# jojolebarjos/board-game-simulator-python

Hardware: AMD Instinct MI355X
Metric: env-steps/sec, Connect4(6,7,4) random rollout, batch=2^20 per GPU (higher is better)
Workload: dtype u64

## Files before the change

### board-game-simulator-python_amd/csrc/bgs_host.hip

```cpp
#include <immintrin.h>
#include <limits.h>
#include <linux/futex.h>
#include <pthread.h>
#include <sched.h>
#include <sys/syscall.h>
#include <time.h>
#include <unistd.h>

#include <atomic>
#include <chrono>
#include <condition_variable>
#include <cstdlib>
#include <cstdio>
#include <algorithm>
#include <cstring>
#include <mutex>
#include <new>
#include <thread>
#include <vector>

#include "bgs_capi_util.h"
#include "bgs_common.h"
#include "bgs_internal.h"

struct bgs_event {
    int device;
    hipEvent_t ev;
};

namespace {

using bgs::fail;

struct ExpandTable {
    uint64_t pairs[256];
    ExpandTable() {
        for (int byte = 0; byte < 256; ++byte) {
            uint64_t four = 0;
            for (int j = 0; j < 4; ++j) four |= (uint64_t)bgs::reward_pair((uint32_t)(byte >> (2 * j)) & 3u) << (16 * j);
            pairs[byte] = four;
        }
    }
};
const ExpandTable g_expand;

template <bool STREAM>
__attribute__((target("avx2"))) int64_t expand_avx2(const uint8_t* src, int64_t code_bytes, int8_t* dst) {
    const __m256i spread = _mm256_setr_epi8(0, 0, 0, 0, 1, 1, 1, 1, 2, 2, 2, 2, 3, 3, 3, 3,
                                            4, 4, 4, 4, 5, 5, 5, 5, 6, 6, 6, 6, 7, 7, 7, 7);
    const __m256i field = _mm256_set1_epi32((int)0xC0300C03u);
    const __m256i one = _mm256_set1_epi32(0x40100401);
    const __m256i two = _mm256_set1_epi32((int)0x80200802u);
    int64_t i = 0;
    for (; i + 8 <= code_bytes; i += 8) {
        long long eight;
        memcpy(&eight, src + i, 8);
        const __m256i rep = _mm256_shuffle_epi8(_mm256_set1_epi64x(eight), spread);
        const __m256i f = _mm256_and_si256(rep, field);
        const __m256i is1 = _mm256_cmpeq_epi8(f, one), is2 = _mm256_cmpeq_epi8(f, two);
        const __m256i r0 = _mm256_sub_epi8(is2, is1), r1 = _mm256_sub_epi8(is1, is2);
        const __m256i lo = _mm256_unpacklo_epi8(r0, r1), hi = _mm256_unpackhi_epi8(r0, r1);
        const __m256i first = _mm256_permute2x128_si256(lo, hi, 0x20), second = _mm256_permute2x128_si256(lo, hi, 0x31);
        if (STREAM) {
            _mm256_stream_si256(reinterpret_cast<__m256i*>(dst + 8 * i), first);
            _mm256_stream_si256(reinterpret_cast<__m256i*>(dst + 8 * i + 32), second);
        } else {
            _mm256_storeu_si256(reinterpret_cast<__m256i*>(dst + 8 * i), first);
            _mm256_storeu_si256(reinterpret_cast<__m256i*>(dst + 8 * i + 32), second);
        }
    }
    if (STREAM) _mm_sfence();
    return i;
}

const bool g_have_avx2 = __builtin_cpu_supports("avx2");
const bool g_stream_stores = bgs::experiment("no_stream_stores") == nullptr;

void expand_range(const uint8_t* packed, int64_t first, int64_t count, int8_t* reward) {
    const int64_t whole = count / 4;
    const uint8_t* src = packed + first / 4;
    int8_t* out = reward + 2 * first;
    int64_t i0 = 0;
    if (g_have_avx2) {
        const bool stream = (reinterpret_cast<uintptr_t>(out) & 31u) == 0 && whole >= (1 << 14) && g_stream_stores;
        i0 = stream ? expand_avx2<true>(src, whole, out) : expand_avx2<false>(src, whole, out);
    }
    for (int64_t i = i0; i < whole; ++i) memcpy(out + 8 * i, &g_expand.pairs[src[i]], 8);
    for (int64_t g = first + whole * 4; g < first + count; ++g) {
        const uint16_t pair = bgs::reward_pair((uint32_t)(packed[g / 4] >> (2 * (g & 3))) & 3u);
        memcpy(reward + 2 * g, &pair, 2);
    }
}

struct CellFormat {
    int cells = 0;
    int nwc = 0;
    int sets = 0;
    int offset = 0;
    int weight[4] = {0, 0, 0, 0};
};

struct SpreadTable {
    uint64_t v[256];
    SpreadTable() {
        for (int byte = 0; byte < 256; ++byte) {
            uint64_t w = 0;
            for (int b = 0; b < 8; ++b) w |= (uint64_t)((byte >> b) & 1) << (8 * b);
            v[byte] = w;
        }
    }
};
const SpreadTable g_spread;

__attribute__((target("avx512f,avx512bw"))) void expand_cells_avx512(const uint64_t* wire, int64_t n, const CellFormat& f,
                                                                      int64_t first, int64_t count, int8_t* out) {
    const __m512i base = _mm512_set1_epi8((char)f.offset);
    __m512i weight[4];
    for (int p = 0; p < f.sets; ++p) weight[p] = _mm512_set1_epi8((char)f.weight[p]);
    alignas(64) int8_t block[64 * 256 + 64];
    const bool lines = f.cells <= 256 && g_stream_stores && (reinterpret_cast<uintptr_t>(out) & 63u) == 0;
#define BGS_ONE_GAME(i_)                                                                                              \
    do {                                                                                                                \
        int8_t* dst_ = out + (i_)*f.cells;                                                                              \
        for (int j = 0; j < f.nwc; ++j) {                                                                               \
// ... 87 lines not shown
    if (!f) return false;
    int node = -1;
    const int got = fscanf(f, "%d", &node);
    fclose(f);
    if (got != 1 || node < 0) return false;
    snprintf(path, sizeof path, "/sys/devices/system/node/node%d/cpulist", node);
    f = fopen(path, "r");
    if (!f) return false;
    char list[4096] = {0};
    const bool have = fgets(list, sizeof list, f) != nullptr;
    fclose(f);
    if (!have) return false;
    cpu_set_t allowed;
    if (sched_getaffinity(0, sizeof allowed, &allowed) != 0) return false;
    int any = 0;
    char* save = nullptr;
    for (char* tok = strtok_r(list, ",\n", &save); tok; tok = strtok_r(nullptr, ",\n", &save)) {
        int lo = 0, hi = 0;
        const int k = sscanf(tok, "%d-%d", &lo, &hi);
        if (k < 1) continue;
        if (k == 1) hi = lo;
        for (int c = lo; c <= hi && c < CPU_SETSIZE; ++c)
            if (CPU_ISSET(c, &allowed)) {
                CPU_SET(c, out);
                ++any;
            }
    }
    return any > 0;
}

}

namespace {
inline bool sink_trace_on() {
    static const bool on = bgs::experiment("sink_trace") != nullptr;
    return on;
}
inline double mono_us() {
    return std::chrono::duration<double, std::micro>(std::chrono::steady_clock::now().time_since_epoch()).count();
}
}

static bool codes_hold_a_zero(const uint8_t* codes, int64_t first, int64_t count) {
    const uint8_t* p = codes + first / 4;
    const int64_t whole = count / 4;
    int64_t i = 0;
    uint64_t seen = 0;
    for (; i + 8 <= whole; i += 8) {
        uint64_t x;
        memcpy(&x, p + i, 8);
        seen |= ~(x | (x >> 1)) & 0x5555555555555555ull;
    }
    for (; i < whole; ++i) seen |= (uint64_t)(~(p[i] | (p[i] >> 1)) & 0x55u);
    for (int64_t k = 0; k < count - whole * 4; ++k) seen |= ((p[whole] >> (2 * k)) & 3u) == 0u ? 1u : 0u;
    return seen != 0;
}

struct bgs_reward_sink {
    int device = 0;
    int64_t max_games = 0;
    int slots = 0;
    int ring = 0;
    int threads = 0;
    std::vector<uint8_t*> pinned;
    std::vector<uint8_t*> mapped;
    std::vector<hipEvent_t> landed;
    bool grids = false;
    CellFormat cells;
    size_t slot_bytes = 0;
    struct Job {
        int64_t n_games = 0;
        int8_t* host_reward = nullptr;
        int event_slot = 0;
        bool all_end = false;
    };
    std::vector<Job> jobs;
    std::mutex mu;
    std::condition_variable cv_submit;
    std::condition_variable cv_landed;
    std::condition_variable cv_done;
    int64_t claimed = 0;
    int64_t submitted = 0;
    volatile int64_t* progress = nullptr;
    int64_t landed_upto = 0;
    int64_t completed = 0;
    std::vector<int> parts_done;
    std::vector<char> slot_ok;
    bool stop = false;
    std::vector<int64_t> failed_tickets;
    bool poll = false;
    std::vector<std::thread> workers;
    std::atomic<int64_t> a_submitted{0}, a_landed{0}, a_completed{0};
    std::atomic<bool> a_stop{false};
    std::atomic<int> urgent{0};
    int spin_us = 0;
    int wait_spin_us = 200;

    bool spin_for(const std::atomic<int64_t>& counter, int64_t ticket) const {
        if (counter.load(std::memory_order_acquire) > ticket) return true;
        if (spin_us <= 0) return false;
        const auto until = std::chrono::steady_clock::now() + std::chrono::microseconds(spin_us);
        for (;;) {
            for (int i = 0; i < 64; ++i) {
                if (counter.load(std::memory_order_acquire) > ticket || a_stop.load(std::memory_order_relaxed)) return true;
                _mm_pause();
            }
            if (std::chrono::steady_clock::now() >= until) return false;
        }
    }

    void work(int t) {
        (void)hipSetDevice(device);
        for (int64_t ticket = 0;; ++ticket) {
            const int slot = (int)(ticket % ring);
            Job job;
            bool ok = true;
            if (t == 0) {
                spin_for(a_submitted, ticket);
                {
                    std::unique_lock<std::mutex> lock(mu);
                    cv_submit.wait(lock, [&] { return stop || submitted > ticket; });
                    if (submitted <= ticket) return;
                    job = jobs[slot];
                }
                if (job.n_games == 0) {
                    ok = false;
                } else if (poll || urgent.load(std::memory_order_relaxed) > 0) {
                    hipError_t e;
                    while ((e = hipEventQuery(landed[job.event_slot])) == hipErrorNotReady) _mm_pause();
                    ok = e == hipSuccess;
                } else {
                    ok = hipEventSynchronize(landed[job.event_slot]) == hipSuccess;
                }
                if (sink_trace_on()) fprintf(stderr, "sink-trace ticket %lld landed %.1f\n", (long long)ticket, mono_us());
                {
                    std::lock_guard<std::mutex> lock(mu);
                    if (!ok && job.n_games != 0) failed_tickets.push_back(ticket);
                    slot_ok[slot] = ok;
                    landed_upto = ticket + 1;
                    a_landed.store(ticket + 1, std::memory_order_release);
                }
                cv_landed.notify_all();
            } else {
                if (urgent.load(std::memory_order_relaxed) > 0) {
                    const auto until = std::chrono::steady_clock::now() + std::chrono::microseconds(2000);
                    while (a_landed.load(std::memory_order_acquire) <= ticket && !a_stop.load(std::memory_order_relaxed) &&
                           urgent.load(std::memory_order_relaxed) > 0 && std::chrono::steady_clock::now() < until)
                        for (int i = 0; i < 16; ++i) _mm_pause();
                } else {
                    spin_for(a_landed, ticket);
                }
                std::unique_lock<std::mutex> lock(mu);
                cv_landed.wait(lock, [&] { return stop || landed_upto > ticket; });
                if (landed_upto <= ticket) return;
                job = jobs[slot];
                ok = slot_ok[slot];
            }
            const int expanders = threads > 1 ? threads - 1 : 1;
            const int share = threads > 1 ? t - 1 : 0;
            if (threads > 1 && t == 0) continue;
            const double trace_t0 = sink_trace_on() ? mono_us() : 0.0;
            if (ok && grids) {
                const int64_t blocks = (job.n_games + 63) / 64;
                const int64_t g0 = blocks * share / expanders * 64;
                const int64_t g1 = share + 1 == expanders ? job.n_games : blocks * (share + 1) / expanders * 64;
                static const bool skip = bgs::experiment("grid_no_expand") != nullptr;
                if (g1 > g0 && !skip) expand_cells(pinned[slot], job.n_games, cells, g0, g1 - g0, job.host_reward);
            } else if (ok) {
                const int64_t bytes = (job.n_games + 3) / 4;
                const int64_t b0 = bytes * share / expanders, b1 = bytes * (share + 1) / expanders;
                const int64_t first = b0 * 4;
                int64_t count = b1 * 4 - first;
                if (first + count > job.n_games) count = job.n_games - first;
                if (count > 0) expand_range(pinned[slot], first, count, job.host_reward);
                if (count > 0 && job.all_end && codes_hold_a_zero(pinned[slot], first, count)) {
                    std::lock_guard<std::mutex> lock(mu);
                    if (std::find(failed_tickets.begin(), failed_tickets.end(), ticket) == failed_tickets.end()) failed_tickets.push_back(ticket);
                }
            }
            if (sink_trace_on()) fprintf(stderr, "sink-trace ticket %lld worker %d expand %.1f .. %.1f\n", (long long)ticket, t, trace_t0, mono_us());
            {
                std::lock_guard<std::mutex> lock(mu);
                if (++parts_done[slot] == expanders) {
                    parts_done[slot] = 0;
                    ++completed;
                    a_completed.store(completed, std::memory_order_release);
                    cv_done.notify_all();
                    if (progress) progress_store_max(progress, completed);
                }
            }
        }
    }
};

namespace {

int64_t claim(bgs_reward_sink* s, bool ahead = false) {
    const int bound = ahead ? s->ring : s->slots;
    s->spin_for(s->a_completed, s->a_submitted.load(std::memory_order_relaxed) - bound);
    std::unique_lock<std::mutex> lock(s->mu);
    s->cv_done.wait(lock, [&] { return s->claimed - s->completed < bound; });
    return s->claimed++;
}

void publish(bgs_reward_sink* s, int64_t ticket, int64_t n_games, int8_t* host_reward, bool ok = true, int64_t event_ticket = -1,
             bool all_end = false) {
    {
        std::unique_lock<std::mutex> lock(s->mu);
        s->cv_done.wait(lock, [&] { return s->submitted == ticket; });
        s->jobs[ticket % s->ring].n_games = ok ? n_games : 0;
        s->jobs[ticket % s->ring].all_end = all_end;
        s->jobs[ticket % s->ring].host_reward = host_reward;
        s->jobs[ticket % s->ring].event_slot = (int)((event_ticket >= 0 ? event_ticket : ticket) % s->ring);
        if (!ok) s->failed_tickets.push_back(ticket);
        s->submitted = ticket + 1;
        s->a_submitted.store(ticket + 1, std::memory_order_release);
    }
    s->cv_submit.notify_one();
    s->cv_done.notify_all();
}

}

namespace bgs {
int64_t sink_claim(bgs_reward_sink* s) { return claim(s); }
uint8_t* sink_slot_device(bgs_reward_sink* s, int64_t ticket) { return s->mapped[ticket % s->ring]; }
uint8_t* sink_slot_host(bgs_reward_sink* s, int64_t ticket) { return s->pinned[ticket % s->ring]; }
hipEvent_t sink_slot_event(bgs_reward_sink* s, int64_t ticket) { return s->landed[ticket % s->ring]; }
void sink_publish(bgs_reward_sink* s, int64_t ticket, int64_t n_games, int8_t* host_reward, bool ok, int64_t event_ticket, bool all_end) {
    publish(s, ticket, n_games, host_reward, ok, event_ticket, all_end);
}
bool sink_takes_group(const bgs_reward_sink* s, int count) { return s != nullptr && !s->grids && count <= s->ring; }
int sink_ring(const bgs_reward_sink* s) { return s->ring; }
int sink_rollout_group(bgs_reward_sink* s, bgs_batch* const* bs, const uint64_t* seeds, const bool* writes, int count,
                       hipStream_t stream, int8_t* const* host_rewards, int64_t* tickets) {
    NEED(count >= 1 && count <= kConnectGroupMax && count <= s->ring && !s->grids, "bad step group");
    for (int i = 0; i < count; ++i)
        NEED(bs[i]->device == s->device && bs[i]->n <= s->max_games, "the batch does not fit the sink");
    uint32_t* codes[kConnectGroupMax];
    for (int i = 0; i < count; ++i) {
        tickets[i] = claim(s, true);
        codes[i] = reinterpret_cast<uint32_t*>(s->mapped[tickets[i] % s->ring]);
    }
    connect_rollout_steps(bs, seeds, codes, writes, count, stream);
    hipError_t err = hipGetLastError();
    if (err == hipSuccess) err = hipEventRecord(s->landed[tickets[count - 1] % s->ring], stream);
    for (int i = 0; i < count; ++i) publish(s, tickets[i], bs[i]->n, host_rewards[i], err == hipSuccess, tickets[count - 1]);
    if (err != hipSuccess) return fail(BGS_ERR_RUNTIME, "grouped rollout could not be enqueued: %s", hipGetErrorString(err));
    return BGS_OK;
}
int sink_wait(bgs_reward_sink* s, int64_t ticket, bool urgent) {
    NEED(s != nullptr, "sink is NULL");
    NEED(ticket >= 0 && ticket < s->a_submitted.load(std::memory_order_acquire), "unknown ticket %lld", (long long)ticket);
    if (s->a_completed.load(std::memory_order_acquire) <= ticket) {
        if (urgent) {
            s->urgent.fetch_add(1, std::memory_order_relaxed);
            const auto until = std::chrono::steady_clock::now() + std::chrono::microseconds(s->wait_spin_us);
            while (s->a_completed.load(std::memory_order_acquire) <= ticket && std::chrono::steady_clock::now() < until)
                for (int i = 0; i < 32; ++i) _mm_pause();
        } else {
            s->spin_for(s->a_completed, ticket);
        }
        {
            std::unique_lock<std::mutex> lock(s->mu);
            s->cv_done.wait(lock, [&] { return s->completed > ticket; });
        }
        if (urgent) s->urgent.fetch_sub(1, std::memory_order_relaxed);
    }
    int64_t bad = -1;
    {
        std::lock_guard<std::mutex> lock(s->mu);
        auto& f = s->failed_tickets;
        for (size_t i = 0; i < f.size();) {
            if (f[i] <= ticket) {
                if (bad < 0 || f[i] < bad) bad = f[i];
                f.erase(f.begin() + (long)i);
            } else {
                ++i;
            }
        }
    }
    if (bad >= 0)
        return fail(BGS_ERR_RUNTIME, "reward hand-over %lld failed (its enqueue, its arrival event, or -- a gathered step whose games all "
                    "had to end -- a rank delivered games that are still running: its step failed there); later deliveries are unaffected",
                    (long long)bad);
    return BGS_OK;
}
}

extern "C" {

int bgs_host_alloc(size_t bytes, void** host_ptr) {
    NEED(host_ptr != nullptr && bytes > 0, "bad argument");
    *host_ptr = nullptr;
    HIP_TRY(hipHostMalloc(host_ptr, bytes, hipHostMallocDefault));
    return BGS_OK;
}

int bgs_host_free(void* host_ptr) {
    if (host_ptr) HIP_TRY(hipHostFree(host_ptr));
    return BGS_OK;
}

int bgs_stream_create(int device, void** hip_stream) {
    NEED(hip_stream != nullptr, "hip_stream is NULL");
    *hip_stream = nullptr;
    int rc = enter_device(device);
    if (rc) return rc;
    hipStream_t s = nullptr;
    HIP_TRY(hipStreamCreateWithFlags(&s, hipStreamNonBlocking));
    *hip_stream = s;
    return BGS_OK;
}

int bgs_stream_destroy(int device, void* hip_stream) {
    if (!hip_stream) return BGS_OK;
    int rc = enter_device(device);
// ... 83 lines not shown
static int make_sink(int device, int64_t max_games, int slots, int threads, size_t slot_bytes, const CellFormat* cells,
                     bgs_reward_sink** out) {
    NEED(out != nullptr, "out is NULL");
    *out = nullptr;
    NEED(max_games >= 1 && slots >= 1 && slots <= 256 && threads >= 1 && threads <= 256,
         "need max_games >= 1, 1 <= slots <= 256, 1 <= threads <= 256");
    int rc = enter_device(device);
    if (rc) return rc;
    bgs_reward_sink* s = new (std::nothrow) bgs_reward_sink();
    NEED(s != nullptr, "out of host memory");
    s->device = device;
    s->max_games = max_games;
    s->slot_bytes = slot_bytes;
    if (cells) {
        s->grids = true;
        s->cells = *cells;
    }
    s->slots = slots;
    s->ring = cells ? slots : std::max(slots, bgs::kSinkGroupRing);
    const int ring = s->ring;
    s->threads = threads;
    s->jobs.resize(ring);
    if (const char* env = bgs::experiment("sink_poll")) s->poll = atoi(env) != 0;
    if (const char* env = bgs::experiment("sink_wait_spin_us")) {
        const int v = atoi(env);
        if (v >= 0 && v <= 1000000) s->wait_spin_us = v;
    }
    if (const char* env = bgs::experiment("sink_spin_us")) {
        const int v = atoi(env);
        if (v >= 0 && v <= 1000000) s->spin_us = v;
    }
    s->parts_done.assign(ring, 0);
    s->slot_ok.assign(ring, 1);
    const size_t bytes = slot_bytes;
    hipError_t err = hipSuccess;
    const char* aff0 = getenv("BGS_SINK_AFFINITY");
    const bool place = !(aff0 && atoi(aff0) == 0);
    cpu_set_t node_cpus, caller_cpus;
    const bool moved = place && device_node_cpus(device, &node_cpus) && sched_getaffinity(0, sizeof caller_cpus, &caller_cpus) == 0 &&
                       sched_setaffinity(0, sizeof node_cpus, &node_cpus) == 0;
    for (int k = 0; k < ring && err == hipSuccess; ++k) {
        void* host = nullptr;
        void* dev = nullptr;
        hipEvent_t ev = nullptr;
        err = hipHostMalloc(&host, bytes, hipHostMallocMapped);
        if (err == hipSuccess) s->pinned.push_back(static_cast<uint8_t*>(host));
        if (err == hipSuccess) err = hipHostGetDevicePointer(&dev, host, 0);
        if (err == hipSuccess) s->mapped.push_back(static_cast<uint8_t*>(dev));
        if (err == hipSuccess) err = hipEventCreateWithFlags(&ev, hipEventDisableTiming);
        if (err == hipSuccess) s->landed.push_back(ev);
    }
    if (moved) (void)sched_setaffinity(0, sizeof caller_cpus, &caller_cpus);
    if (err != hipSuccess) {
        for (auto p : s->pinned) (void)hipHostFree(p);
        for (auto e : s->landed) (void)hipEventDestroy(e);
        delete s;
        return fail(BGS_ERR_RUNTIME, "reward sink allocation failed: %s", hipGetErrorString(err));
    }
    for (int t = 0; t < threads; ++t) s->workers.emplace_back([s, t] { s->work(t); });
    const char* aff = getenv("BGS_SINK_AFFINITY");
    cpu_set_t cpus;
    if (!(aff && atoi(aff) == 0) && device_node_cpus(device, &cpus))
        for (auto& w : s->workers) (void)pthread_setaffinity_np(w.native_handle(), sizeof cpus, &cpus);
    *out = s;
    return BGS_OK;
}

int bgs_sink_create(int device, int64_t max_games, int slots, int threads, bgs_reward_sink** out) {
    NEED(max_games >= 1, "max_games must be >= 1");
    return make_sink(device, max_games, slots, threads, (size_t)(max_games + 63) / 64 * 16, nullptr, out);
}

static CellFormat cell_format(const bgs_batch* b) {
    CellFormat f;
    const int h = b->generic ? b->gen_h : (b->game == BGS_GAME_CONNECT ? b->cg.h : b->bg.h);
    const int w = b->generic ? b->gen_w : (b->game == BGS_GAME_CONNECT ? b->cg.w : b->bg.w);
    f.cells = h * w;
    if (b->generic) return f;
    f.nwc = (f.cells + 63) / 64;
// ... 138 lines not shown
    {
        std::unique_lock<std::mutex> lock(s->mu);
        s->cv_done.wait(lock, [&] { return s->completed == s->claimed; });
        s->stop = true;
        s->a_stop.store(true, std::memory_order_release);
    }
    s->cv_submit.notify_all();
    s->cv_landed.notify_all();
    for (auto& w : s->workers) w.join();
    (void)hipSetDevice(s->device);
    for (auto p : s->pinned) (void)hipHostFree(p);
    for (auto e : s->landed) (void)hipEventDestroy(e);
    delete s;
    return BGS_OK;
}

int bgs_sink_submit(bgs_reward_sink* s, bgs_batch* b, int8_t* host_reward, int64_t* ticket) {
    NEED(s != nullptr && b != nullptr && host_reward != nullptr, "NULL argument");
    NEED(b->device == s->device, "batch lives on device %d, the sink on device %d", b->device, s->device);
    NEED(b->n <= s->max_games, "batch of %lld games exceeds the sink's %lld", (long long)b->n, (long long)s->max_games);
    int rc = enter_device(s->device);
    if (rc) return rc;
    if (s->grids && (rc = grid_sink_matches(s, b))) return rc;
    const int64_t t = claim(s);
    const int slot = (int)(t % s->ring);
    hipError_t err;
    if (s->grids) {
        err = enqueue_grids(s, b, slot);
    } else {
        bgs::pack_outcomes(b, s->mapped[slot]);
        err = hipGetLastError();
    }
    if (err == hipSuccess) err = hipEventRecord(s->landed[slot], b->stream);
    publish(s, t, b->n, host_reward, err == hipSuccess);
    if (ticket) *ticket = t;
    if (err != hipSuccess) return fail(BGS_ERR_RUNTIME, "reward hand-over could not be enqueued: %s", hipGetErrorString(err));
    return BGS_OK;
}

int bgs_sink_rollout(bgs_reward_sink* s, bgs_batch* b, uint64_t seed, int32_t max_plies, uint32_t flags,
                     int8_t* host_reward, int64_t* ticket) {
    NEED(s != nullptr && b != nullptr && host_reward != nullptr, "NULL argument");
    NEED(b->device == s->device, "batch lives on device %d, the sink on device %d", b->device, s->device);
    NEED(b->n <= s->max_games, "batch of %lld games exceeds the sink's %lld", (long long)b->n, (long long)s->max_games);
    if (s->grids) {
        int rc0 = grid_sink_matches(s, b);
        if (rc0) return rc0;
    }
    NEED(max_plies >= 0, "max_plies must be >= 0");
    {
        int rc0 = enter_device(s->device);
        if (rc0) return rc0;
    }
    const int64_t t = claim(s);
    const int slot = (int)(t % s->ring);
    int rc = s->grids ? bgs_rollout(b, seed, max_plies, flags) : bgs::rollout_with_codes(b, seed, max_plies, flags, s->mapped[slot]);
    hipError_t err = hipSuccess;
    if (rc == BGS_OK && s->grids) err = enqueue_grids(s, b, slot);
    if (rc == BGS_OK && err == hipSuccess) err = hipEventRecord(s->landed[slot], b->stream);
    publish(s, t, b->n, host_reward, rc == BGS_OK && err == hipSuccess);
    if (ticket) *ticket = t;
    if (rc) return rc;
    if (err != hipSuccess) return fail(BGS_ERR_RUNTIME, "reward hand-over could not be enqueued: %s", hipGetErrorString(err));
    return BGS_OK;
}

int bgs_sink_submit_packed(bgs_reward_sink* s, void* hip_stream, const void* device_packed, int64_t n_games,
                           int8_t* host_reward, int64_t* ticket) {
    NEED(s != nullptr && device_packed != nullptr && host_reward != nullptr, "NULL argument");
    NEED(!s->grids, "a grid sink takes boards (bgs_sink_submit / bgs_sink_rollout), not outcome codes");
    NEED(n_games >= 1 && n_games <= s->max_games, "n_games %lld outside 1..%lld", (long long)n_games,
         (long long)s->max_games);
    int rc = enter_device(s->device);
    if (rc) return rc;
    hipStream_t stream = static_cast<hipStream_t>(hip_stream);
    const int64_t t = claim(s);
    const int slot = (int)(t % s->ring);
    hipError_t err = hipMemcpyAsync(s->pinned[slot], device_packed, (size_t)(n_games + 3) / 4, hipMemcpyDeviceToHost, stream);
    if (err == hipSuccess) err = hipEventRecord(s->landed[slot], stream);
    publish(s, t, n_games, host_reward, err == hipSuccess);
    if (ticket) *ticket = t;
    if (err != hipSuccess) return fail(BGS_ERR_RUNTIME, "reward hand-over could not be enqueued: %s", hipGetErrorString(err));
    return BGS_OK;
}

int bgs_sink_wait(bgs_reward_sink* s, int64_t ticket) { return bgs::sink_wait(s, ticket, false); }

}
```

### board-game-simulator-python_amd/csrc/bgs_internal.h

```cpp
#pragma once

#include <hip/hip_runtime.h>
#include <stdint.h>
#include <stddef.h>

struct bgs_reward_sink;
struct bgs_gather;

enum { BGS_GAME_CONNECT = 1, BGS_GAME_BOUNCE = 2 };

#include "connect_unit.h"
#include "bounce_unit.h"

struct bgs_batch {
    int game;
    int generic;
    int gen_h, gen_w, gen_k;
    uint32_t gen_init_status;
    int device;
    int64_t n;
    hipStream_t stream;
    uint64_t first_game;
    ConnectGeom cg;
    BounceGeom bg;
// ... 124 lines not shown
                       int8_t* d_winner, int32_t* d_plies, uint64_t* d_targets, int8_t* d_reward_out, uint32_t* d_done = nullptr,
                       uint32_t ticket = 0);
void bounce_rollout(const bgs_batch* b, uint64_t seed, int32_t max_plies, uint32_t flags);
int bounce_book_acquire(bgs_batch* b, int max_depth);
void bounce_book_release(bgs_batch* b);
void bounce_unpack_grid(const bgs_batch* b, int8_t* d_grid);
void bounce_meta(const bgs_batch* b, int8_t* d_player, uint8_t* d_ended, int8_t* d_winner, int32_t* d_plies);
void bounce_targets(const bgs_batch* b, uint64_t* d_targets, int32_t* d_count);
void bounce_pack(const bgs_batch* b, const int8_t* d_grid, const int8_t* d_player, const int8_t* d_winner,
                 const int32_t* d_plies, int32_t* d_status_out);

size_t generic_bounce_legal_bytes(int h, int w);
void generic_reset(const bgs_batch* b);
void generic_play(const bgs_batch* b, uint64_t seed, uint32_t max_plies, uint32_t count, bool from_initial, bool per_ply = false);
void generic_step_actions(const bgs_batch* b, const int32_t* d_actions, int32_t* d_status_out);
void generic_unpack_grid(const bgs_batch* b, int8_t* d_grid);
void generic_meta(const bgs_batch* b, int8_t* d_player, uint8_t* d_ended, int8_t* d_winner, int32_t* d_plies);
void generic_connect_legal(const bgs_batch* b, uint8_t* d_legal, int32_t* d_count);
void generic_bounce_targets(const bgs_batch* b, uint8_t* d_wide, int32_t* d_count);
void generic_pack(const bgs_batch* b, const int8_t* d_grid, const int8_t* d_player, const int8_t* d_winner,
                  const int32_t* d_plies, int32_t* d_status_out);

void pack_outcomes(const bgs_batch* b, uint8_t* d_packed);
int rollout_with_codes(bgs_batch* b, uint64_t seed, int32_t max_plies, uint32_t flags, uint8_t* codes_out);


int64_t sink_claim(bgs_reward_sink* s);
uint8_t* sink_slot_device(bgs_reward_sink* s, int64_t ticket);
uint8_t* sink_slot_host(bgs_reward_sink* s, int64_t ticket);
hipEvent_t sink_slot_event(bgs_reward_sink* s, int64_t ticket);
void sink_publish(bgs_reward_sink* s, int64_t ticket, int64_t n_games, int8_t* host_reward, bool ok, int64_t event_ticket = -1,
                  bool all_end = false);
int sink_wait(bgs_reward_sink* s, int64_t ticket, bool urgent);
constexpr int kSinkGroupRing = 4 * kConnectGroupMax;
bool sink_takes_group(const bgs_reward_sink* s, int count);
int sink_ring(const bgs_reward_sink* s);
int sink_rollout_group(bgs_reward_sink* s, bgs_batch* const* bs, const uint64_t* seeds, const bool* writes, int count,
                       hipStream_t stream, int8_t* const* host_rewards, int64_t* tickets);
int gather_wait(bgs_gather* g, int64_t ticket, bool urgent);

}
```

### board-game-simulator-python_amd/csrc/bgs_pipeline.hip

```cpp
#include <cstdlib>
#include <new>
#include <atomic>
#include <chrono>
#include <condition_variable>
#include <deque>
#include <memory>
#include <mutex>
#include <thread>
#include <immintrin.h>
#include <string>
#include <vector>

#include "bgs_capi_util.h"
#include "bgs_common.h"
#include "bgs_internal.h"
#include "connect_group_plan.h"

using bgs::fail;

struct StreamSyncer {
    std::thread th;
    std::mutex mu;
    std::condition_variable cv;
    int cmd = 0;
// ... 18 lines not shown
        stream = s;
        done.store(0, std::memory_order_relaxed);
        { std::lock_guard<std::mutex> lock(mu); cmd = 1; }
        cv.notify_one();
    }
    bool wait() {
        for (int spins = 0; !done.load(std::memory_order_acquire); ++spins) {
            if (spins < 20000) _mm_pause();
            else std::this_thread::sleep_for(std::chrono::microseconds(50));
        }
        return err.exchange(0) == 0;
    }
};

struct bgs_pipeline {
    int device = 0;
    std::vector<bgs_batch*> batches;
    bgs_reward_sink* sink = nullptr;
    bgs_gather* gather = nullptr;
    std::vector<int8_t*> host;
    std::vector<int64_t> ticket;
    std::vector<int64_t> held;
    uint64_t seed0 = 0;
    int32_t max_plies = 0x7FFFFFFF;
    uint32_t flags = BGS_ROLLOUT_FROM_INITIAL;
    int64_t step = 0;
    int64_t handed = 0;
    const int64_t* rank_words = nullptr;
    int64_t word_stride = 8;
    int world = 1;
    int64_t* consumed = nullptr;
    bool consumer = false;
    int lag = 0;
    int64_t timeout_ms = 60000;
    std::vector<std::unique_ptr<StreamSyncer>> syncers;
    std::vector<hipEvent_t> ev0, ev1;
    size_t brackets = 0;
    std::mutex mu;
    std::condition_variable cv;
    std::thread feeder;
    std::deque<uint64_t> fed;
    int64_t fed_end = 0;
    int64_t released = 0;
    bool feeding = false;
    bool stop = false;
    int feed_rc = BGS_OK;
    std::string feed_error;
    std::vector<hipEvent_t> start_ev, end_ev;
    int64_t launches = 0;
};

extern "C" {

int bgs_pipeline_create(bgs_batch* const* batches, int depth, bgs_reward_sink* sink, bgs_gather* gather,
                        int8_t* const* host_rewards, int n_host, uint64_t seed0, int32_t max_plies, uint32_t flags,
                        bgs_pipeline** out) {
    NEED(out != nullptr && batches != nullptr, "NULL argument");
    *out = nullptr;
    NEED(depth >= 1 && depth <= 64, "depth must be in 1..64");
    NEED(!(sink && gather), "a pipeline hands over through a sink OR a gather");
    NEED(max_plies >= 0, "max_plies must be >= 0");
    NEED((sink || gather) ? (host_rewards != nullptr && n_host >= 1 && n_host <= 256) : n_host == 0,
         "a hand-over needs 1..256 host arrays, a pipeline without one takes none");
    for (int k = 0; k < depth; ++k) {
        NEED(batches[k] != nullptr, "batch %d is NULL", k);
        NEED(batches[k]->device == batches[0]->device && batches[k]->n == batches[0]->n, "the batches must be alike");
        for (int j = 0; j < k; ++j) NEED(batches[j] != batches[k], "batch %d is listed twice", k);
    }
    bgs_pipeline* p = new (std::nothrow) bgs_pipeline();
    NEED(p != nullptr, "out of host memory");
    p->device = batches[0]->device;
    p->batches.assign(batches, batches + depth);
    for (bgs_batch* b : p->batches) b->launches_in_flight = depth;
    p->sink = sink;
    p->gather = gather;
    for (int h = 0; h < n_host; ++h) p->host.push_back(host_rewards[h]);
    p->ticket.assign(n_host, -1);
    p->held.assign(n_host, -1);
    p->seed0 = seed0;
    p->max_plies = max_plies;
    p->flags = flags;
    *out = p;
    return BGS_OK;
}

int bgs_pipeline_set_ring(bgs_pipeline* p, const int64_t* rank_words, int64_t word_stride, int world, int64_t* consumed,
                          int is_consumer, int lag, int64_t timeout_ms) {
    NEED(p != nullptr, "pipeline is NULL");
    NEED(rank_words == nullptr || (world >= 1 && word_stride >= 1 && consumed != nullptr), "bad ring description");
    NEED(!is_consumer || (lag >= 1 && lag < (int)p->host.size()),
         "the consumer trails the launches by 1 .. (host arrays - 1) hand-overs");
    p->rank_words = rank_words;
    p->word_stride = word_stride;
    p->world = world;
    p->consumed = consumed;
    p->consumer = is_consumer != 0;
    p->lag = lag;
    p->timeout_ms = timeout_ms;
    return BGS_OK;
}

static int wait_ticket(bgs_pipeline* p, int64_t t, bool urgent = false) {
    return p->sink ? bgs::sink_wait(p->sink, t, urgent) : bgs::gather_wait(p->gather, t, urgent);
}

static int consume(bgs_pipeline* p, int64_t j) {
    int rc = bgs_progress_wait(p->rank_words, p->world, p->word_stride, j + 1, p->timeout_ms, nullptr);
    if (rc) return rc;
    return bgs_progress_store(p->consumed, j + 1);
}

static int group_size(const bgs_pipeline* p, int64_t count, int handover, bool from_feeder) {
    int s = count >= kConnectGroupMinCall ? kConnectGroupSteps : 1;
    if (const char* e = bgs::experiment("connect_group")) s = atoi(e);
    if (s > kConnectGroupMax) s = kConnectGroupMax;
    if (s < 2 || from_feeder || p->rank_words) return 1;
    if (handover && (p->gather || !bgs::sink_takes_group(p->sink, s) || (int)p->host.size() < s)) return 1;
    for (const bgs_batch* b : p->batches)
        if (!bgs::connect_steps_ok(b, p->max_plies, p->flags, handover != 0)) return 1;
    return s;
}

static int enqueue_steps(bgs_pipeline* p, const uint64_t* seeds, int64_t count, int handover, int time_stride, bool from_feeder = false) {
    NEED(p != nullptr && count >= 0, "bad argument");
    NEED(!handover || p->sink || p->gather, "this pipeline has no hand-over");
    std::unique_lock<std::mutex> lock(p->mu);
    const bool fed_pending = p->feeding && p->handed < p->fed_end && p->feed_rc == BGS_OK;
    lock.unlock();
    NEED(from_feeder || !fed_pending, "steps are being fed to this pipeline (bgs_pipeline_feed): enqueue when they have all been consumed");
    HIP_TRY(hipSetDevice(p->device));
    const int depth = (int)p->batches.size();
// ... 360 lines not shown
```

Measured before the change: 1042 billion.

## Expand reward codes in band as they land instead of waiting on event

For grouped rollouts, the sink workers no longer wait on a landed event. They poll the mapped pinned buffer in 128-byte units and expand each unit as soon as it holds no zero codes, so host expansion overlaps the GPU kernel writing codes. The buffer is zeroed after each use so that zero can mark unwritten data. A grace timeout with a stream query handles codes that never land. This adds spinning CPU polling, extra zeroing, and a dependency on nonzero codes as the sentinel.

```diff
diff --git a/board-game-simulator-python_amd/csrc/bgs_host.hip b/board-game-simulator-python_amd/csrc/bgs_host.hip
--- a/board-game-simulator-python_amd/csrc/bgs_host.hip
+++ b/board-game-simulator-python_amd/csrc/bgs_host.hip
@@ -14,6 +14,7 @@
 #include <cstdio>
 #include <algorithm>
 #include <cstring>
+#include <memory>
 #include <mutex>
 #include <new>
 #include <thread>
@@ -22,6 +23,7 @@
 #include "bgs_capi_util.h"
 #include "bgs_common.h"
 #include "bgs_internal.h"
+#include "sink_codes.h"
 
 struct bgs_event {
     int device;
@@ -32,64 +34,10 @@
 
 using bgs::fail;
 
-struct ExpandTable {
-    uint64_t pairs[256];
-    ExpandTable() {
-        for (int byte = 0; byte < 256; ++byte) {
-            uint64_t four = 0;
-            for (int j = 0; j < 4; ++j) four |= (uint64_t)bgs::reward_pair((uint32_t)(byte >> (2 * j)) & 3u) << (16 * j);
-            pairs[byte] = four;
-        }
-    }
-};
-const ExpandTable g_expand;
-
-template <bool STREAM>
-__attribute__((target("avx2"))) int64_t expand_avx2(const uint8_t* src, int64_t code_bytes, int8_t* dst) {
-    const __m256i spread = _mm256_setr_epi8(0, 0, 0, 0, 1, 1, 1, 1, 2, 2, 2, 2, 3, 3, 3, 3,
-                                            4, 4, 4, 4, 5, 5, 5, 5, 6, 6, 6, 6, 7, 7, 7, 7);
-    const __m256i field = _mm256_set1_epi32((int)0xC0300C03u);
-    const __m256i one = _mm256_set1_epi32(0x40100401);
-    const __m256i two = _mm256_set1_epi32((int)0x80200802u);
-    int64_t i = 0;
-    for (; i + 8 <= code_bytes; i += 8) {
-        long long eight;
-        memcpy(&eight, src + i, 8);
-        const __m256i rep = _mm256_shuffle_epi8(_mm256_set1_epi64x(eight), spread);
-        const __m256i f = _mm256_and_si256(rep, field);
-        const __m256i is1 = _mm256_cmpeq_epi8(f, one), is2 = _mm256_cmpeq_epi8(f, two);
-        const __m256i r0 = _mm256_sub_epi8(is2, is1), r1 = _mm256_sub_epi8(is1, is2);
-        const __m256i lo = _mm256_unpacklo_epi8(r0, r1), hi = _mm256_unpackhi_epi8(r0, r1);
-        const __m256i first = _mm256_permute2x128_si256(lo, hi, 0x20), second = _mm256_permute2x128_si256(lo, hi, 0x31);
-        if (STREAM) {
-            _mm256_stream_si256(reinterpret_cast<__m256i*>(dst + 8 * i), first);
-            _mm256_stream_si256(reinterpret_cast<__m256i*>(dst + 8 * i + 32), second);
-        } else {
-            _mm256_storeu_si256(reinterpret_cast<__m256i*>(dst + 8 * i), first);
-            _mm256_storeu_si256(reinterpret_cast<__m256i*>(dst + 8 * i + 32), second);
-        }
-    }
-    if (STREAM) _mm_sfence();
-    return i;
-}
-
-const bool g_have_avx2 = __builtin_cpu_supports("avx2");
 const bool g_stream_stores = bgs::experiment("no_stream_stores") == nullptr;
 
 void expand_range(const uint8_t* packed, int64_t first, int64_t count, int8_t* reward) {
-    const int64_t whole = count / 4;
-    const uint8_t* src = packed + first / 4;
-    int8_t* out = reward + 2 * first;
-    int64_t i0 = 0;
-    if (g_have_avx2) {
-        const bool stream = (reinterpret_cast<uintptr_t>(out) & 31u) == 0 && whole >= (1 << 14) && g_stream_stores;
-        i0 = stream ? expand_avx2<true>(src, whole, out) : expand_avx2<false>(src, whole, out);
-    }
-    for (int64_t i = i0; i < whole; ++i) memcpy(out + 8 * i, &g_expand.pairs[src[i]], 8);
-    for (int64_t g = first + whole * 4; g < first + count; ++g) {
-        const uint16_t pair = bgs::reward_pair((uint32_t)(packed[g / 4] >> (2 * (g & 3))) & 3u);
-        memcpy(reward + 2 * g, &pair, 2);
-    }
+    sink_codes::expand_range(packed, first, count, reward, g_stream_stores);
 }
 
 struct CellFormat {
@@ -243,29 +191,13 @@
 }
 
 namespace {
-inline bool sink_trace_on() {
-    static const bool on = bgs::experiment("sink_trace") != nullptr;
-    return on;
-}
+inline bool sink_trace_on() { return bgs::experiment("sink_trace") != nullptr; }
 inline double mono_us() {
     return std::chrono::duration<double, std::micro>(std::chrono::steady_clock::now().time_since_epoch()).count();
 }
 }
 
-static bool codes_hold_a_zero(const uint8_t* codes, int64_t first, int64_t count) {
-    const uint8_t* p = codes + first / 4;
-    const int64_t whole = count / 4;
-    int64_t i = 0;
-    uint64_t seen = 0;
-    for (; i + 8 <= whole; i += 8) {
-        uint64_t x;
-        memcpy(&x, p + i, 8);
-        seen |= ~(x | (x >> 1)) & 0x5555555555555555ull;
-    }
-    for (; i < whole; ++i) seen |= (uint64_t)(~(p[i] | (p[i] >> 1)) & 0x55u);
-    for (int64_t k = 0; k < count - whole * 4; ++k) seen |= ((p[whole] >> (2 * k)) & 3u) == 0u ? 1u : 0u;
-    return seen != 0;
-}
+using sink_codes::codes_hold_a_zero;
 
 struct bgs_reward_sink {
     int device = 0;
@@ -284,6 +216,9 @@
         int8_t* host_reward = nullptr;
         int event_slot = 0;
         bool all_end = false;
+        bool inband = false;
+        hipStream_t stream = nullptr;
+        int64_t code_bytes = 0;
     };
     std::vector<Job> jobs;
     std::mutex mu;
@@ -300,6 +235,11 @@
     bool stop = false;
     std::vector<int64_t> failed_tickets;
     bool poll = false;
+    bool trace = false;
+    bool inband_on = true;
+    std::atomic<int64_t> grace_ms{bgs::kHandoverTimeoutMs};
+    std::unique_ptr<std::atomic<int>[]> inband_failed;
+    static constexpr int64_t kInbandSpinUs = 200, kInbandSleepUs = 50;
     std::vector<std::thread> workers;
     std::atomic<int64_t> a_submitted{0}, a_landed{0}, a_completed{0};
     std::atomic<bool> a_stop{false};
@@ -318,6 +258,48 @@
             }
             if (std::chrono::steady_clock::now() >= until) return false;
         }
+    }
+
+    void take_inband(int64_t ticket, int slot, const Job& job, int64_t b0, int64_t b1, int t) {
+        using clock = std::chrono::steady_clock;
+        const bool stream_stores = g_stream_stores && b1 - b0 >= (1 << 14);
+        const double trace_t0 = trace ? mono_us() : 0.0;
+        double trace_missing = 0.0;
+        int64_t at = b0;
+        auto progress_at = clock::now();
+        while (at < b1 && !inband_failed[slot].load(std::memory_order_acquire)) {
+            const int64_t got = sink_codes::take_landed(pinned[slot], at, b1, job.n_games, job.host_reward, stream_stores);
+            if (got == b1) {
+                at = got;
+                break;
+            }
+            const auto now = clock::now();
+            if (trace) trace_missing = mono_us();
+            if (got != at) {
+                at = got;
+                progress_at = now;
+                continue;
+            }
+            const int64_t idle_us = std::chrono::duration_cast<std::chrono::microseconds>(now - progress_at).count();
+            if (idle_us >= grace_ms.load(std::memory_order_relaxed) * 1000) {
+                const hipError_t e = hipStreamQuery(job.stream);
+                if (e == hipErrorNotReady) {
+                    progress_at = now;
+                    continue;
+                }
+                if (e == hipSuccess) at = sink_codes::take_landed(pinned[slot], at, b1, job.n_games, job.host_reward, stream_stores);
+                if (at < b1) {
+                    std::lock_guard<std::mutex> lock(mu);
+                    if (std::find(failed_tickets.begin(), failed_tickets.end(), ticket) == failed_tickets.end()) failed_tickets.push_back(ticket);
+                    inband_failed[slot].store(1, std::memory_order_release);
+                }
+                break;
+            }
+            if (idle_us >= kInbandSpinUs) std::this_thread::sleep_for(std::chrono::microseconds(kInbandSleepUs));
+            else for (int i = 0; i < 16; ++i) _mm_pause();
+        }
+        if (trace)
+            fprintf(stderr, "sink-trace ticket %lld worker %d inband %.1f .. %.1f missing %.1f\n", (long long)ticket, t, trace_t0, mono_us(), trace_missing);
     }
 
     void work(int t) {
@@ -336,6 +318,7 @@
                 }
                 if (job.n_games == 0) {
                     ok = false;
+                } else if (job.inband) {
                 } else if (poll || urgent.load(std::memory_order_relaxed) > 0) {
                     hipError_t e;
                     while ((e = hipEventQuery(landed[job.event_slot])) == hipErrorNotReady) _mm_pause();
@@ -343,7 +326,7 @@
                 } else {
                     ok = hipEventSynchronize(landed[job.event_slot]) == hipSuccess;
                 }
-                if (sink_trace_on()) fprintf(stderr, "sink-trace ticket %lld landed %.1f\n", (long long)ticket, mono_us());
+                if (trace) fprintf(stderr, "sink-trace ticket %lld %s %.1f\n", (long long)ticket, job.inband ? "passed" : "landed", mono_us());
                 {
                     std::lock_guard<std::mutex> lock(mu);
                     if (!ok && job.n_games != 0) failed_tickets.push_back(ticket);
@@ -370,32 +353,39 @@
             const int expanders = threads > 1 ? threads - 1 : 1;
             const int share = threads > 1 ? t - 1 : 0;
             if (threads > 1 && t == 0) continue;
-            const double trace_t0 = sink_trace_on() ? mono_us() : 0.0;
+            const double trace_t0 = trace ? mono_us() : 0.0;
             if (ok && grids) {
                 const int64_t blocks = (job.n_games + 63) / 64;
                 const int64_t g0 = blocks * share / expanders * 64;
                 const int64_t g1 = share + 1 == expanders ? job.n_games : blocks * (share + 1) / expanders * 64;
                 static const bool skip = bgs::experiment("grid_no_expand") != nullptr;
                 if (g1 > g0 && !skip) expand_cells(pinned[slot], job.n_games, cells, g0, g1 - g0, job.host_reward);
-            } else if (ok) {
-                const int64_t bytes = (job.n_games + 3) / 4;
-                const int64_t b0 = bytes * share / expanders, b1 = bytes * (share + 1) / expanders;
-                const int64_t first = b0 * 4;
-                int64_t count = b1 * 4 - first;
-                if (first + count > job.n_games) count = job.n_games - first;
-                if (count > 0) expand_range(pinned[slot], first, count, job.host_reward);
-                if (count > 0 && job.all_end && codes_hold_a_zero(pinned[slot], first, count)) {
-                    std::lock_guard<std::mutex> lock(mu);
-                    if (std::find(failed_tickets.begin(), failed_tickets.end(), ticket) == failed_tickets.end()) failed_tickets.push_back(ticket);
+            } else if (!grids) {
+                int64_t b0, b1;
+                sink_codes::share_of(job.code_bytes, share, expanders, &b0, &b1);
+                if (ok && job.inband) {
+                    take_inband(ticket, slot, job, b0, b1, t);
+                } else if (ok) {
+                    const int64_t first = b0 * 4;
+                    const int64_t count = (b1 * 4 < job.n_games ? b1 * 4 : job.n_games) - first;
+                    if (count > 0) expand_range(pinned[slot], first, count, job.host_reward);
+                    if (count > 0 && job.all_end && codes_hold_a_zero(pinned[slot], first, count)) {
+                        std::lock_guard<std::mutex> lock(mu);
+                        if (std::find(failed_tickets.begin(), failed_tickets.end(), ticket) == failed_tickets.end()) failed_tickets.push_back(ticket);
+                    }
                 }
-            }
-            if (sink_trace_on()) fprintf(stderr, "sink-trace ticket %lld worker %d expand %.1f .. %.1f\n", (long long)ticket, t, trace_t0, mono_us());
+                sink_codes::zero_share(pinned[slot], b0, b1);
+            }
+            if (trace && !(ok && job.inband && !grids))
+                fprintf(stderr, "sink-trace ticket %lld worker %d expand %.1f .. %.1f\n", (long long)ticket, t, trace_t0, mono_us());
             {
                 std::lock_guard<std::mutex> lock(mu);
                 if (++parts_done[slot] == expanders) {
                     parts_done[slot] = 0;
+                    inband_failed[slot].store(0, std::memory_order_relaxed);
                     ++completed;
                     a_completed.store(completed, std::memory_order_release);
+                    if (trace) fprintf(stderr, "sink-trace ticket %lld completed %.1f\n", (long long)ticket, mono_us());
                     cv_done.notify_all();
                     if (progress) progress_store_max(progress, completed);
                 }
@@ -415,12 +405,15 @@
 }
 
 void publish(bgs_reward_sink* s, int64_t ticket, int64_t n_games, int8_t* host_reward, bool ok = true, int64_t event_ticket = -1,
-             bool all_end = false) {
+             bool all_end = false, bool inband = false, hipStream_t inband_stream = nullptr) {
     {
         std::unique_lock<std::mutex> lock(s->mu);
         s->cv_done.wait(lock, [&] { return s->submitted == ticket; });
         s->jobs[ticket % s->ring].n_games = ok ? n_games : 0;
         s->jobs[ticket % s->ring].all_end = all_end;
+        s->jobs[ticket % s->ring].inband = inband;
+        s->jobs[ticket % s->ring].stream = inband_stream;
+        s->jobs[ticket % s->ring].code_bytes = s->grids ? 0 : (n_games + 3) / 4;
         s->jobs[ticket % s->ring].host_reward = host_reward;
         s->jobs[ticket % s->ring].event_slot = (int)((event_ticket >= 0 ? event_ticket : ticket) % s->ring);
         if (!ok) s->failed_tickets.push_back(ticket);
@@ -429,6 +422,16 @@
     }
     s->cv_submit.notify_one();
     s->cv_done.notify_all();
+}
+
+inline bool skip_launch(int64_t ticket) {
+#ifdef BGS_TEST_HOOKS
+    const char* e = bgs::experiment("sink_skip_launch");
+    return e != nullptr && atoll(e) == ticket;
+#else
+    (void)ticket;
+    return false;
+#endif
 }
 
 }
@@ -443,6 +446,9 @@
 }
 bool sink_takes_group(const bgs_reward_sink* s, int count) { return s != nullptr && !s->grids && count <= s->ring; }
 int sink_ring(const bgs_reward_sink* s) { return s->ring; }
+void sink_set_grace_ms(bgs_reward_sink* s, int64_t grace_ms) {
+    if (s != nullptr && grace_ms >= 1 && bgs::experiment("sink_grace_ms") == nullptr) s->grace_ms.store(grace_ms, std::memory_order_relaxed);
+}
 int sink_rollout_group(bgs_reward_sink* s, bgs_batch* const* bs, const uint64_t* seeds, const bool* writes, int count,
                        hipStream_t stream, int8_t* const* host_rewards, int64_t* tickets) {
     NEED(count >= 1 && count <= kConnectGroupMax && count <= s->ring && !s->grids, "bad step group");
@@ -453,10 +459,17 @@
         tickets[i] = claim(s, true);
         codes[i] = reinterpret_cast<uint32_t*>(s->mapped[tickets[i] % s->ring]);
     }
-    connect_rollout_steps(bs, seeds, codes, writes, count, stream);
-    hipError_t err = hipGetLastError();
-    if (err == hipSuccess) err = hipEventRecord(s->landed[tickets[count - 1] % s->ring], stream);
-    for (int i = 0; i < count; ++i) publish(s, tickets[i], bs[i]->n, host_rewards[i], err == hipSuccess, tickets[count - 1]);
+    hipError_t err = hipSuccess;
+    if (!skip_launch(tickets[0])) {
+        connect_rollout_steps(bs, seeds, codes, writes, count, stream);
+        err = hipGetLastError();
+    }
+    const bool inband = s->inband_on;
+    if (err == hipSuccess && !inband) err = hipEventRecord(s->landed[tickets[count - 1] % s->ring], stream);
+    if (err != hipSuccess) (void)hipStreamSynchronize(stream);
+    for (int i = 0; i < count; ++i)
+        publish(s, tickets[i], bs[i]->n, host_rewards[i], err == hipSuccess, tickets[count - 1], false, inband, stream);
+    if (s->trace) fprintf(stderr, "sink-trace launch tickets %lld .. %lld\n", (long long)tickets[0], (long long)tickets[count - 1]);
     if (err != hipSuccess) return fail(BGS_ERR_RUNTIME, "grouped rollout could not be enqueued: %s", hipGetErrorString(err));
     return BGS_OK;
 }
@@ -492,8 +505,9 @@
         }
     }
     if (bad >= 0)
-        return fail(BGS_ERR_RUNTIME, "reward hand-over %lld failed (its enqueue, its arrival event, or -- a gathered step whose games all "
-                    "had to end -- a rank delivered games that are still running: its step failed there); later deliveries are unaffected",
+        return fail(BGS_ERR_RUNTIME, "reward hand-over %lld failed (its enqueue, its arrival event, a step in band whose codes never landed, or -- a "
+                    "gathered step whose games all had to end -- a rank delivered games that are still running: its step failed there); "
+                    "later deliveries are unaffected",
                     (long long)bad);
     return BGS_OK;
 }
@@ -643,6 +657,14 @@
     }
     s->parts_done.assign(ring, 0);
     s->slot_ok.assign(ring, 1);
+    s->inband_failed.reset(new std::atomic<int>[ring]);
+    for (int k = 0; k < ring; ++k) s->inband_failed[k].store(0, std::memory_order_relaxed);
+    s->trace = sink_trace_on();
+    if (const char* env = bgs::experiment("sink_inband")) s->inband_on = atoi(env) != 0;
+    if (const char* env = bgs::experiment("sink_grace_ms")) {
+        const long long v = atoll(env);
+        if (v >= 1 && v <= 3600000) s->grace_ms.store(v);
+    }
     const size_t bytes = slot_bytes;
     hipError_t err = hipSuccess;
     const char* aff0 = getenv("BGS_SINK_AFFINITY");
@@ -656,6 +678,7 @@
         hipEvent_t ev = nullptr;
         err = hipHostMalloc(&host, bytes, hipHostMallocMapped);
         if (err == hipSuccess) s->pinned.push_back(static_cast<uint8_t*>(host));
+        if (err == hipSuccess && !cells) memset(host, 0, bytes);
         if (err == hipSuccess) err = hipHostGetDevicePointer(&dev, host, 0);
         if (err == hipSuccess) s->mapped.push_back(static_cast<uint8_t*>(dev));
         if (err == hipSuccess) err = hipEventCreateWithFlags(&ev, hipEventDisableTiming);
@@ -860,6 +883,7 @@
         err = hipGetLastError();
     }
     if (err == hipSuccess) err = hipEventRecord(s->landed[slot], b->stream);
+    if (err != hipSuccess) (void)hipStreamSynchronize(b->stream);
     publish(s, t, b->n, host_reward, err == hipSuccess);
     if (ticket) *ticket = t;
     if (err != hipSuccess) return fail(BGS_ERR_RUNTIME, "reward hand-over could not be enqueued: %s", hipGetErrorString(err));
@@ -882,11 +906,15 @@
     }
     const int64_t t = claim(s);
     const int slot = (int)(t % s->ring);
-    int rc = s->grids ? bgs_rollout(b, seed, max_plies, flags) : bgs::rollout_with_codes(b, seed, max_plies, flags, s->mapped[slot]);
+    const bool inband = !s->grids && s->inband_on && bgs::connect_steps_ok(b, max_plies, flags, true);
+    int rc = BGS_OK;
+    if (!(inband && skip_launch(t)))
+        rc = s->grids ? bgs_rollout(b, seed, max_plies, flags) : bgs::rollout_with_codes(b, seed, max_plies, flags, s->mapped[slot]);
     hipError_t err = hipSuccess;
     if (rc == BGS_OK && s->grids) err = enqueue_grids(s, b, slot);
-    if (rc == BGS_OK && err == hipSuccess) err = hipEventRecord(s->landed[slot], b->stream);
-    publish(s, t, b->n, host_reward, rc == BGS_OK && err == hipSuccess);
+    if (rc == BGS_OK && err == hipSuccess && !inband) err = hipEventRecord(s->landed[slot], b->stream);
+    if (rc != BGS_OK || err != hipSuccess) (void)hipStreamSynchronize(b->stream);
+    publish(s, t, b->n, host_reward, rc == BGS_OK && err == hipSuccess, -1, false, inband, b->stream);
     if (ticket) *ticket = t;
     if (rc) return rc;
     if (err != hipSuccess) return fail(BGS_ERR_RUNTIME, "reward hand-over could not be enqueued: %s", hipGetErrorString(err));
@@ -906,6 +934,7 @@
     const int slot = (int)(t % s->ring);
     hipError_t err = hipMemcpyAsync(s->pinned[slot], device_packed, (size_t)(n_games + 3) / 4, hipMemcpyDeviceToHost, stream);
     if (err == hipSuccess) err = hipEventRecord(s->landed[slot], stream);
+    if (err != hipSuccess) (void)hipStreamSynchronize(stream);
     publish(s, t, n_games, host_reward, err == hipSuccess);
     if (ticket) *ticket = t;
     if (err != hipSuccess) return fail(BGS_ERR_RUNTIME, "reward hand-over could not be enqueued: %s", hipGetErrorString(err));
diff --git a/board-game-simulator-python_amd/csrc/bgs_internal.h b/board-game-simulator-python_amd/csrc/bgs_internal.h
--- a/board-game-simulator-python_amd/csrc/bgs_internal.h
+++ b/board-game-simulator-python_amd/csrc/bgs_internal.h
@@ -180,6 +180,8 @@
 void sink_publish(bgs_reward_sink* s, int64_t ticket, int64_t n_games, int8_t* host_reward, bool ok, int64_t event_ticket = -1,
                   bool all_end = false);
 int sink_wait(bgs_reward_sink* s, int64_t ticket, bool urgent);
+constexpr int64_t kHandoverTimeoutMs = 60000;
+void sink_set_grace_ms(bgs_reward_sink* s, int64_t grace_ms);
 constexpr int kSinkGroupRing = 4 * kConnectGroupMax;
 bool sink_takes_group(const bgs_reward_sink* s, int count);
 int sink_ring(const bgs_reward_sink* s);
diff --git a/board-game-simulator-python_amd/csrc/bgs_pipeline.hip b/board-game-simulator-python_amd/csrc/bgs_pipeline.hip
--- a/board-game-simulator-python_amd/csrc/bgs_pipeline.hip
+++ b/board-game-simulator-python_amd/csrc/bgs_pipeline.hip
@@ -74,7 +74,7 @@
     int64_t* consumed = nullptr;
     bool consumer = false;
     int lag = 0;
-    int64_t timeout_ms = 60000;
+    int64_t timeout_ms = bgs::kHandoverTimeoutMs;
     std::vector<std::unique_ptr<StreamSyncer>> syncers;
     std::vector<hipEvent_t> ev0, ev1;
     size_t brackets = 0;
@@ -139,6 +139,7 @@
     p->consumer = is_consumer != 0;
     p->lag = lag;
     p->timeout_ms = timeout_ms;
+    if (p->sink) bgs::sink_set_grace_ms(p->sink, timeout_ms);
     return BGS_OK;
 }
 
diff --git a/board-game-simulator-python_amd/csrc/sink_codes.h b/board-game-simulator-python_amd/csrc/sink_codes.h
--- /dev/null
+++ b/board-game-simulator-python_amd/csrc/sink_codes.h
@@ -0,0 +1,148 @@
+#pragma once
+
+#include <immintrin.h>
+#include <stdint.h>
+#include <string.h>
+
+namespace sink_codes {
+
+constexpr uint16_t pair_of(uint32_t code) { return code == 1u ? (uint16_t)0xFF01u : code == 2u ? (uint16_t)0x01FFu : (uint16_t)0u; }
+
+struct ExpandTable {
+    uint64_t pairs[256];
+    ExpandTable() {
+        for (int byte = 0; byte < 256; ++byte) {
+            uint64_t four = 0;
+            for (int j = 0; j < 4; ++j) four |= (uint64_t)pair_of((uint32_t)(byte >> (2 * j)) & 3u) << (16 * j);
+            pairs[byte] = four;
+        }
+    }
+};
+inline const ExpandTable& table() {
+    static const ExpandTable t;
+    return t;
+}
+inline bool have_avx2() {
+    static const bool have = __builtin_cpu_supports("avx2");
+    return have;
+}
+
+template <bool STREAM>
+__attribute__((target("avx2"), always_inline)) inline void expand8_avx2(long long eight, int8_t* dst) {
+    const __m256i spread = _mm256_setr_epi8(0, 0, 0, 0, 1, 1, 1, 1, 2, 2, 2, 2, 3, 3, 3, 3,
+                                            4, 4, 4, 4, 5, 5, 5, 5, 6, 6, 6, 6, 7, 7, 7, 7);
+    const __m256i field = _mm256_set1_epi32((int)0xC0300C03u);
+    const __m256i one = _mm256_set1_epi32(0x40100401);
+    const __m256i two = _mm256_set1_epi32((int)0x80200802u);
+    const __m256i rep = _mm256_shuffle_epi8(_mm256_set1_epi64x(eight), spread);
+    const __m256i f = _mm256_and_si256(rep, field);
+    const __m256i is1 = _mm256_cmpeq_epi8(f, one), is2 = _mm256_cmpeq_epi8(f, two);
+    const __m256i r0 = _mm256_sub_epi8(is2, is1), r1 = _mm256_sub_epi8(is1, is2);
+    const __m256i lo = _mm256_unpacklo_epi8(r0, r1), hi = _mm256_unpackhi_epi8(r0, r1);
+    const __m256i first = _mm256_permute2x128_si256(lo, hi, 0x20), second = _mm256_permute2x128_si256(lo, hi, 0x31);
+    if (STREAM) {
+        _mm256_stream_si256(reinterpret_cast<__m256i*>(dst), first);
+        _mm256_stream_si256(reinterpret_cast<__m256i*>(dst + 32), second);
+    } else {
+        _mm256_storeu_si256(reinterpret_cast<__m256i*>(dst), first);
+        _mm256_storeu_si256(reinterpret_cast<__m256i*>(dst + 32), second);
+    }
+}
+template <bool STREAM>
+__attribute__((target("avx2"))) inline int64_t expand_avx2(const uint8_t* src, int64_t code_bytes, int8_t* dst) {
+    int64_t i = 0;
+    for (; i + 8 <= code_bytes; i += 8) {
+        long long eight;
+        memcpy(&eight, src + i, 8);
+        expand8_avx2<STREAM>(eight, dst + 8 * i);
+    }
+    if (STREAM) _mm_sfence();
+    return i;
+}
+
+inline void expand_range(const uint8_t* packed, int64_t first, int64_t count, int8_t* reward, bool stream_stores = true) {
+    const int64_t whole = count / 4;
+    const uint8_t* src = packed + first / 4;
+    int8_t* out = reward + 2 * first;
+    int64_t i0 = 0;
+    if (have_avx2()) {
+        const bool stream = (reinterpret_cast<uintptr_t>(out) & 31u) == 0 && whole >= (1 << 14) && stream_stores;
+        i0 = stream ? expand_avx2<true>(src, whole, out) : expand_avx2<false>(src, whole, out);
+    }
+    for (int64_t i = i0; i < whole; ++i) memcpy(out + 8 * i, &table().pairs[src[i]], 8);
+    for (int64_t g = first + whole * 4; g < first + count; ++g) {
+        const uint16_t pair = pair_of((uint32_t)(packed[g / 4] >> (2 * (g & 3))) & 3u);
+        memcpy(reward + 2 * g, &pair, 2);
+    }
+}
+
+inline bool codes_hold_a_zero(const uint8_t* codes, int64_t first, int64_t count) {
+    const uint8_t* p = codes + first / 4;
+    const int64_t whole = count / 4;
+    int64_t i = 0;
+    uint64_t seen = 0;
+    for (; i + 8 <= whole; i += 8) {
+        uint64_t x;
+        memcpy(&x, p + i, 8);
+        seen |= ~(x | (x >> 1)) & 0x5555555555555555ull;
+    }
+    for (; i < whole; ++i) seen |= (uint64_t)(~(p[i] | (p[i] >> 1)) & 0x55u);
+    for (int64_t k = 0; k < count - whole * 4; ++k) seen |= ((p[whole] >> (2 * k)) & 3u) == 0u ? 1u : 0u;
+    return seen != 0;
+}
+
+constexpr int64_t kInbandUnit = 128;
+
+inline void share_of(int64_t bytes, int share, int expanders, int64_t* b0, int64_t* b1) {
+    const int64_t units = (bytes + kInbandUnit - 1) / kInbandUnit;
+    const int64_t u0 = units * share / expanders * kInbandUnit, u1 = units * (share + 1) / expanders * kInbandUnit;
+    *b0 = u0 < bytes ? u0 : bytes;
+    *b1 = u1 < bytes ? u1 : bytes;
+}
+
+template <bool STREAM>
+__attribute__((target("avx2"))) inline bool take_unit_avx2(const uint8_t* src, int8_t* dst) {
+    const __m256i fives = _mm256_set1_epi8(0x55);
+    __m256i v[4];
+    for (int k = 0; k < 4; ++k) v[k] = _mm256_loadu_si256(reinterpret_cast<const __m256i*>(src + 32 * k));
+    __asm__ __volatile__("" : "+x"(v[0]), "+x"(v[1]), "+x"(v[2]), "+x"(v[3]) : : "memory");
+    __m256i all = fives;
+    for (int k = 0; k < 4; ++k) all = _mm256_and_si256(all, _mm256_or_si256(v[k], _mm256_srli_epi16(v[k], 1)));
+    if (_mm256_movemask_epi8(_mm256_cmpeq_epi8(all, fives)) != -1) return false;
+    for (int k = 0; k < 4; ++k) {
+        alignas(32) long long w[4];
+        _mm256_store_si256(reinterpret_cast<__m256i*>(w), v[k]);
+        for (int j = 0; j < 4; ++j) expand8_avx2<STREAM>(w[j], dst + 8 * (32 * k + 8 * j));
+    }
+    return true;
+}
+
+inline int64_t take_landed(const uint8_t* slot, int64_t from, int64_t b1, int64_t n, int8_t* reward, bool stream_stores) {
+    const bool avx2 = have_avx2();
+    const bool stream = stream_stores && (reinterpret_cast<uintptr_t>(reward) & 31u) == 0;
+    int64_t b = from;
+    bool streamed = false;
+    while (b < b1) {
+        const int64_t e = b + kInbandUnit < b1 ? b + kInbandUnit : b1;
+        if (avx2 && e - b == kInbandUnit && 4 * e <= n) {
+            if (!(stream ? take_unit_avx2<true>(slot + b, reward + 8 * b) : take_unit_avx2<false>(slot + b, reward + 8 * b))) break;
+            streamed = stream;
+        } else {
+            uint8_t unit[kInbandUnit];
+            memcpy(unit, slot + b, (size_t)(e - b));
+            __asm__ __volatile__("" : : "r"(unit) : "memory");
+            const int64_t games = (4 * e < n ? 4 * e : n) - 4 * b;
+            if (codes_hold_a_zero(unit, 0, games)) break;
+            expand_range(unit, 0, games, reward + 8 * b, false);
+        }
+        b = e;
+    }
+    if (streamed) _mm_sfence();
+    return b;
+}
+
+inline void zero_share(uint8_t* slot, int64_t b0, int64_t b1) {
+    if (b1 > b0) memset(slot + b0, 0, (size_t)(b1 - b0));
+}
+
+}
```

Measured after the change: 1043 billion (median of 3 runs). About the same (+0.1%).
